# finsberg/fenicsx-beat

Measured on AMD Instinct MI355X. Metric: node_updates_per_sec, higher is better.
Workload: dtype f64

## Files before the change

### fenicsx-beat_amd/beat/_engine.py

```python

from __future__ import annotations

import ctypes as C
import os
from dataclasses import dataclass
from types import SimpleNamespace
from typing import Any

import numpy as np

from . import _hip
from ._deferred import DeferredUpdate


@dataclass
class Slab:

    nz_global: int
    rank: int = 0
    world: int = 1
    weights: Any = None

    def __post_init__(self):
        if self.world > self.nz_global:
# ... 333 lines not shown
        ptrs, amps, k = self._stim_args(stim_w, stim_amp)
        return self.deferred.solved(x, *_solve_record(lambda info, pend: self.lib.beat_pde_solve_dist(
            self.handle, comm.handle, v_prev.ptr, ptrs, amps, k, x.ptr, C.c_void_p(self.work.data_ptr()), rtol, atol, max_it,
            int(defer_flush), info, pend)))

    def set_guess_order(self, order: int) -> None:
        if isinstance(order, str):
            if order != "auto":
                raise ValueError(f"guess order must be an integer 0..4 or 'auto', got {order!r}")
            order = -1
        self.flush_pending()
        _hip.check(self.lib.beat_pde_set_guess_order(self.handle, int(order)))
        self.guess_order = int(order)

    def set_single_reduction(self, on) -> None:
        _hip.check(self.lib.beat_pde_set_single_reduction(self.handle, -1 if on is None else int(bool(on))))

    def set_small(self, enable: bool) -> None:
        _hip.check(self.lib.beat_pde_set_small_grid_solve(self.handle, int(bool(enable))))

    def small_active(self) -> bool:
        return bool(self.lib.beat_pde_small_grid_solve_active(self.handle))

    RR_ROUTE_KEYS = ("available", "ry", "pd", "by_rows_mask", "nsegx", "nrb", "zc", "nchunks", "total_blocks", "guess_ry")

    def rr_route(self) -> dict:
        out = (C.c_int * len(self.RR_ROUTE_KEYS))()
        _hip.check(self.lib.beat_pde_rr_route(self.handle, out))
        return {k: int(v) for k, v in zip(self.RR_ROUTE_KEYS, out)}

    def guess_traffic(self) -> dict:
        out = (C.c_int * 4)()
        _hip.check(self.lib.beat_pde_guess_traffic(self.handle, out))
        return {"reads": int(out[0]), "writes": int(out[1]), "order": int(out[2]), "pending": bool(out[3])}

    def guess_reset(self) -> None:
        self.flush_pending()
        _hip.check(self.lib.beat_pde_guess_reset(self.handle))

    def flush_pending(self) -> None:
        self.deferred.flush()

    def apply(self, which, x, y):
        _hip.check(self.lib.beat_pde_apply(self.handle, which, x.ptr, y.ptr))


def conductivity_array(M, mesh) -> np.ndarray:
    from . import _stencil, grid

    if isinstance(M, (grid.Function, grid.VectorFunction)):
        raise TypeError("the conductivity is a tensor: build it from a fibre field with "
                        "beat.conductivities.define_conductivity_tensor (vector P1 functions and per-cell fields are accepted)")
# ... 462 lines not shown
```

### fenicsx-beat_amd/beat/_hip.py

```python

from __future__ import annotations

import ctypes as C
import os
from pathlib import Path

_HERE = Path(__file__).resolve().parent
_LIB_PATH = Path(os.environ.get("BEAT_HIP_LIBRARY", _HERE / "lib" / "libbeat_hip.so"))

MODEL_SIMPLE_ODE = 0
MODEL_FHN_DEMO = 1
MODEL_FHN_README = 2
MODEL_TP06_GRL1 = 3
MODEL_TORORD_DYNCL_GRL1 = 4
MODEL_TORORD_LAND_GRL1 = 5
(MATH_EXP, MATH_EXP_INT, MATH_LOG, MATH_LOG_INT, MATH_RCP, MATH_RSQRT, MATH_TP06_RCP2, MATH_TP06_RCP3, MATH_TP06_RCP4,
 MATH_TORORD_RCP2, MATH_TORORD_RCP3, MATH_TORORD_RCP4, MATH_TP06_PHI_SMALL, MATH_TP06_PHI7, MATH_TORORD_PHI_SMALL,
 MATH_TORORD_PHI7, MATH_TP06_GRL1, MATH_TP06_ADVANCE, MATH_TP06_GATE, MATH_TORORD_ADVANCE, MATH_TORORD_GATE,
 MATH_TORORD_GATE_B) = range(22)
MATH_IN = (1, 1, 1, 1, 1, 1, 2, 3, 4, 2, 3, 4, 1, 1, 1, 1, 4, 4, 4, 4, 4, 4)
MATH_OUT = (1, 1, 1, 1, 1, 1, 2, 3, 4, 2, 3, 4, 1, 1, 1, 1, 1, 1, 1, 1, 1, 1)
MAX_STIM = 8
MAX_CLASSES = 32
MAX_LEADS = 16
# ... 80 lines not shown
    "beat_pde_set_timestep": (_int, [_vp, _dbl, _dbl, _dbl]),
    "beat_pde_apply": (_int, [_vp, _int, _vp, _vp]),
    "beat_pde_rhs": (_int, [_vp, _vp, C.POINTER(_vp), C.POINTER(_dbl), _int, _vp, _vp, _vp, _vp]),
    "beat_pde_cg_begin": (_int, [_vp, _vp, _dbl, _dbl, _int]),
    "beat_pde_spmv_dot": (_int, [_vp, _vp, _vp, _vp]),
    "beat_pde_spmv_dot_part": (_int, [_vp, _vp, _vp, _vp, _int]),
    "beat_pde_cg_update": (_int, [_vp, _vp, _vp, _vp, _vp, _vp]),
    "beat_pde_cg_next": (_int, [_vp, _vp, _vp, _vp]),
    "beat_pde_ring_size": (_int, []),
    "beat_pde_cg_update_r": (_int, [_vp, _vp, _vp, _vp, _int]),
    "beat_pde_cg_next_oop": (_int, [_vp, _vp, _vp, _vp, _vp]),
    "beat_pde_x_flush": (_int, [_vp, _vp, _vp, _vp, _i64, _int, _int]),
    "beat_pde_set_small_grid_solve": (_int, [_vp, _int]),
    "beat_pde_small_grid_solve_active": (_int, [_vp]),
    "beat_split_steps": (_int, [_vp, _int, _vp, _i64, _i64, _vp, _int, _int, _vp, _int, _vp, _vp, _vp, _vp, _int, _dbl, _dbl,
                                _int, _vp, _vp, _int, _vp, _vp]),
    "beat_split_steps_big": (_int, [_vp, _int, _vp, _i64, _i64, _vp, _int, _int, _vp, _vp, _int, _vp, _vp, _vp, _vp, _int, _dbl, _dbl, _int, _int,
                             C.POINTER(KspInfo), C.POINTER(_int), C.POINTER(C.c_float)]),
    "beat_pde_set_guess_order": (_int, [_vp, _int]),
    "beat_pde_set_single_reduction": (_int, [_vp, _int]),
    "beat_pde_fused_dist_pass": (_int, [_vp]),
    "beat_pde_tile_route": (_int, [_vp]),
    "beat_pde_rr_route": (_int, [_vp, C.POINTER(_int)]),
    "beat_pde_guess_reset": (_int, [_vp]),
    "beat_pde_guess_pending": (_int, [_vp]),
    "beat_pde_guess_history": (_int, [_vp, _vp, _vp, _vp]),
    "beat_pde_guess_traffic": (_int, [_vp, C.POINTER(_int)]),
    "beat_pde_set_preconditioner": (_int, [_vp, _int, _vp]),
    "beat_pde_pc_num_passes": (_int, [_vp]),
    "beat_pde_pc_pass": (_int, [_vp, _int, _vp, _vp, _vp, _vp, _vp]),
    "beat_pde_cg_first_z": (_int, [_vp, _vp, _vp, _vp]),
    "beat_pde_cg_next_z": (_int, [_vp, _vp, _vp, _vp]),
    "beat_pde_work_fields": (_int, [_vp]),
    "beat_pde_field_stride": (_i64, [_vp]),
    "beat_pde_solve": (
        _int,
        [_vp, _vp, C.POINTER(_vp), C.POINTER(_dbl), _int, _vp, _vp, _dbl, _dbl, _int, C.POINTER(KspInfo)],
    ),
    "beat_pde_solve_begin": (_int, [_vp, _vp, C.POINTER(_vp), C.POINTER(_dbl), _int, _vp, _vp, _dbl, _dbl, _int]),
    "beat_pde_solve_end": (_int, [_vp, C.POINTER(KspInfo), C.POINTER(_int)]),
    "beat_pde_solve_is_open": (_int, [_vp]),
    "beat_pde_solve_can_open": (_int, [_vp]),
    "beat_pde_solve_ex": (
        _int,
        [_vp, _vp, C.POINTER(_vp), C.POINTER(_dbl), _int, _vp, _vp, _dbl, _dbl, _int, _int, C.POINTER(KspInfo), C.POINTER(_int)],
    ),
# ... 93 lines not shown
```

### fenicsx-beat_amd/csrc/beat_pde.hip

```cpp
#include "beat_pde_internal.h"
#include "beat_pde_device.h"

#include <algorithm>
#include <cmath>
#include <cstdlib>
#include <cstring>
#include <vector>

const int beat_pde_detail::kOffsets[45] = {0, 0, 0,  1, 0, 0,  -1, 0, 0,  0, 1, 0,  0, -1, 0,  0, 0, 1,  0, 0, -1,
                          1, 1, 0,  -1, -1, 0,  0, 1, 1,  0, -1, -1,  1, 0, 1,  -1, 0, -1,
                          1, 1, 1,  -1, -1, -1};

namespace {
using namespace beat_pde_detail;

template <int TX_, int TY_>
struct Tile {
  static constexpr int TX = TX_, TY = TY_;
  static constexpr int PITCH = TX + 2;
  static constexpr int SLOT = (TY + 2) * PITCH;
  static constexpr int NLOAD = (SLOT + BEAT_BLOCK - 1) / BEAT_BLOCK;
  static constexpr int ROWS_PER_THREAD = TY / (BEAT_BLOCK / TX);
  static_assert(TX * TY == 1024 && ROWS_PER_THREAD == 4, "tile must hold 1024 nodes");
};
// ... 217 lines not shown
    __syncthreads();
  }

  if (MODE == MODE_SPMV_DOT || MODE == MODE_PC) {
    const double s0 = beat_block_sum(acc0, red);
    if (threadIdx.x == 0) a.partials[g.part_off + t] = s0;
  } else if (MODE == MODE_RHS) {
    const double s0 = beat_block_sum(acc0, red);
    const double s1 = beat_block_sum(acc1, red);
    const double s2 = beat_block_sum(acc2, red);
    if (threadIdx.x == 0) {
      a.partials[g.part_off + t] = s0;
      a.partials[BEAT_MAX_PARTIALS + g.part_off + t] = s1;
      a.partials[2 * BEAT_MAX_PARTIALS + g.part_off + t] = s2;
    }
  }
}

__global__ __launch_bounds__(BEAT_BLOCK) void reduce_partials_kernel(const double* __restrict__ partials, int count, int nsum, double* out,
                                                                     const double* st, double* counter, int then, double* roll_st,
                                                                     double rtol, double atol, double max_it, double* alpha_slot,
                                                                     double bound_c) {
  __shared__ double red[4];
  if (st != nullptr && st[STOP] != 0.0) return;
  if (counter != nullptr && threadIdx.x == 0) counter[0] += 1.0;
  for (int k = 0; k < nsum; ++k) {
    double s = 0.0;
    for (int i = threadIdx.x; i < count; i += BEAT_BLOCK) s += partials[(int64_t)k * BEAT_MAX_PARTIALS + i];
    s = beat_block_sum(s, red);
    if (threadIdx.x == 0) out[k] = s;
  }
  if (then != STEP_NONE && threadIdx.x == 0) beat_pcg_step(then, roll_st, rtol, atol, max_it, alpha_slot, bound_c);
}

__global__ void pcg_step_kernel(int kind, double* st, double rtol, double atol, double max_it, double* alpha_slot, double bound_c) {
  beat_pcg_step(kind, st, rtol, atol, max_it, alpha_slot, bound_c);
}

template <bool VAR>
__global__ __launch_bounds__(BEAT_BLOCK) void cg_update_kernel(Geom g, const double* __restrict__ st,
                                                               double* __restrict__ x,
                                                               double* __restrict__ r,
                                                               const double* __restrict__ p,
                                                               const double* __restrict__ q,
                                                               const double* __restrict__ dinv,
                                                               double dinv_i, double* __restrict__ partials) {
  __shared__ double red[4];
  if (st[STOP] != 0.0) return;
  const double alpha = st[RZ] / st[PQ];
  const int lane = threadIdx.x & 63, wave = threadIdx.x >> 6;
  const int nrows = g.ny * g.nz;
  double s_rz = 0.0, s_rr = 0.0;
  for (int row = blockIdx.x * 4 + wave; row < nrows; row += gridDim.x * 4) {
    const int iz = row / g.ny, iy = row - iz * g.ny;
    const int tyz = 3 * axis_type(iy, g.ny, 1, 1) + 9 * axis_type(iz, g.nz, g.z_lo_phys, g.z_hi_phys);
// ... 202 lines not shown
  const int TX = tile_tx, TY = 1024 / tile_tx;
  g.tiles_x = (g.nx + TX - 1) / TX;
  g.tiles_y = (g.ny + TY - 1) / TY;
  const int tiles = g.tiles_x * g.tiles_y;
  int nchunks = std::max(1, (TARGET_BLOCKS + tiles - 1) / tiles);
  nchunks = std::min(nchunks, g.nz);
  g.zc = (g.nz + nchunks - 1) / nchunks;
  g.nchunks = (g.nz + g.zc - 1) / g.zc;
  const int64_t total = (int64_t)tiles * g.nchunks;
  if (total > BEAT_MAX_PARTIALS) {
    g.nchunks = std::max(1, (int)(BEAT_MAX_PARTIALS / tiles));
    g.zc = (g.nz + g.nchunks - 1) / g.nchunks;
    g.nchunks = (g.nz + g.zc - 1) / g.zc;
  }
  BEAT_REQUIRE((int64_t)tiles * g.nchunks <= BEAT_MAX_PARTIALS, "xy plane too large: %d tiles", tiles);
  g.total = tiles * g.nchunks;
  g.z_lo = 0;
  g.z_hi = g.nz;
  g.part_off = 0;
  p->n = n[0] * n[1] * n[2];
  const int64_t rows = (int64_t)g.ny * g.nz;
  p->vec_grid = (unsigned)std::min<int64_t>(2048, std::max<int64_t>(1, (rows + 3) / 4));
  if (const char* e = std::getenv("BEAT_PCG_PREDICT_STOP")) p->predict_stop = e[0] != '0';
  std::memcpy(p->h_mass, host_mass_tab, sizeof(p->h_mass));
  std::memcpy(p->h_stiff, host_stiff_tab, sizeof(p->h_stiff));
  BEAT_HIP_CHECK(hipSetDevice(ctx->device));
  BEAT_HIP_CHECK(hipMalloc(&p->d_tabs, sizeof(double) * (4 * 27 * TABW + 32)));
  BEAT_HIP_CHECK(hipMalloc(&p->d_st, sizeof(double) * BEAT_ST_DOUBLES));
  BEAT_HIP_CHECK(hipMalloc(&p->d_alphas, sizeof(double) * PRING_MAX));
  BEAT_HIP_CHECK(hipMemsetAsync(p->d_st, 0, sizeof(double) * BEAT_ST_DOUBLES, ctx->stream));
  const int rc = upload_tables(p);
  if (rc) return rc;
  *out = p;
  return BEAT_OK;
}


extern "C" int beat_pde_set_ghost_types(beat_pde* pde, int ghost_lo_type, int ghost_hi_type) {
  BEAT_REQUIRE(pde != nullptr, "null pde");
  BEAT_REQUIRE(ghost_lo_type >= 0 && ghost_lo_type <= 2 && ghost_hi_type >= 0 && ghost_hi_type <= 2, "node types are 0, 1 or 2");
  pde->ghost_lo_tz = ghost_lo_type;
  pde->ghost_hi_tz = ghost_hi_type;
  return BEAT_OK;
}

extern "C" int beat_pde_destroy(beat_pde* pde) {
  if (pde == nullptr) return BEAT_OK;
  if (pde->open.on && pde->ctx != nullptr) (void)hipStreamSynchronize(pde->ctx->stream);
  (void)hipFree(pde->d_tabs);
  (void)hipFree(pde->d_st);
  (void)hipFree(pde->d_alphas);
  (void)hipFree(pde->d_batch_st);
  (void)hipFree(pde->guess.alloc);
  if (pde->h_st) (void)hipHostFree(pde->h_st);
  if (pde->ev_st) (void)hipEventDestroy(pde->ev_st);
  (void)hipFree(pde->v_A);
  (void)hipFree(pde->v_dinv);
  (void)hipFree(pde->v_B);
  (void)hipFree(pde->v_gc0);
  (void)hipFree(pde->v_seg);
  (void)hipFree(pde->v_segmask);
  (void)hipFree(pde->v_seg_tiled);
  (void)hipFree(pde->v_segmask_tiled);
  beat_vrr_destroy(pde);
  beat_vtl_destroy(pde);
  delete pde;
  return BEAT_OK;
}

static int upload_tables(beat_pde* pde) {
  const double C_m = pde->C_m, theta = pde->theta, dt = pde->dt;
  std::vector<double> h(4 * 27 * TABW + 32, 0.0);
  for (int t = 0; t < 27; ++t) {
    for (int k = 0; k < 15; ++k) {
// ... 601 lines not shown
```

### fenicsx-beat_amd/csrc/beat_pde_device.h

```cpp
#pragma once

namespace beat_pde_detail {

__device__ __forceinline__ int axis_type(int i, int n, int lo_phys, int hi_phys) {
  if (n == 1 && lo_phys && hi_phys) return 1;
  if (i == 0 && lo_phys) return 0;
  if (i == n - 1 && hi_phys) return 2;
  return 1;
}

__device__ __forceinline__ int xcd_block(int b, int total) {
  const int per = (total + 7) >> 3;
  return (b & 7) * per + (b >> 3);
}

__device__ __forceinline__ double from_left(double v) {
  const int lo = __builtin_amdgcn_update_dpp(0, __double2loint(v), 0x138, 0xf, 0xf, true);
  const int hi = __builtin_amdgcn_update_dpp(0, __double2hiint(v), 0x138, 0xf, 0xf, true);
  return __hiloint2double(hi, lo);
}
__device__ __forceinline__ double from_right(double v) {
  const int lo = __builtin_amdgcn_update_dpp(0, __double2loint(v), 0x130, 0xf, 0xf, true);
  const int hi = __builtin_amdgcn_update_dpp(0, __double2hiint(v), 0x130, 0xf, 0xf, true);
  return __hiloint2double(hi, lo);
}
// ... 12 lines not shown
```

### fenicsx-beat_amd/csrc/beat_pde_internal.h

```cpp
#pragma once
#include "beat_common.h"
#include "beat_pcg_scalar.h"
#include "beat_slab_parts.h"

#include <algorithm>
#include <cstdlib>
#include <vector>

namespace beat_pde_detail {

constexpr int PRING = 6;
constexpr int PRING_MAX = 12;
constexpr int TABW = 16;

extern const int kOffsets[45];

struct Geom {
  int nx, ny, nz;
  int64_t plane;
  int tiles_x, tiles_y, nchunks, zc, total;
  int z_lo_phys, z_hi_phys;
  int tile_tx;
  int z_lo, z_hi;
  int part_off;
// ... 30 lines not shown
  struct OpenSolve {
    bool on = false;
    int kind = beat_pde_detail::SOLVE_RR;
    bool pdot = false;
    double* x = nullptr;
    double* work = nullptr;
    int max_it = 0, launched = 0;
    int limit = 0;
    void* comm = nullptr;
    bool rr = false, merged = false, vpdot = false;
  } open;
  struct Part0 {
    int pass = beat_pde_detail::PASS_NONE;
    int blocks = 0;
  } part0;
  double* h_st = nullptr;
  hipEvent_t ev_st = nullptr;
  beat_ksp_info last_info{};
  int last_rc = 0;
  int ring = beat_pde_detail::PRING;
  int last_base = 0;
  bool predict_stop = true;
  double predict_c = 0.0;
  double* d_batch_st = nullptr;
  int ghost_lo_tz = 1, ghost_hi_tz = 1;
  int single_reduction = -1;
  beat_guess_state guess;
  void* vrr = nullptr;
  void* vtl = nullptr;
  bool small_enabled = true;
  int pc_ncoef = 1;
  double pc_coef[8] = {1.0};
  bool var = false;
  const double* v_mass = nullptr;
  const double* v_stiff = nullptr;
  double* v_A = nullptr;
  double* v_dinv = nullptr;
  double* v_B = nullptr;
  double* v_gc0 = nullptr;
  bool v_gc0_valid = false;
  bool v_pdot_dist = false;
  int64_t v_ld = 0;
  int* v_seg = nullptr;
  std::vector<int> h_seg;
  unsigned long long* v_segmask = nullptr;
  int* v_seg_tiled = nullptr;
// ... 160 lines not shown
```

### fenicsx-beat_amd/csrc/beat_pde_rr.hip

```cpp
#include "beat_pde_internal.h"
#include "beat_pde_device.h"

#include <algorithm>
#include <cmath>
#include <cstddef>
#include <cstdlib>

namespace {
using namespace beat_pde_detail;

constexpr int SEG = 62;

struct Coef {
  double c[15];
};

struct RGeom {
  int nx, ny, nz;
  int64_t plane;
  int ry;
  int nsegx, nrb, nchunks, zc;
  int total_waves, total_blocks;
  int z_lo_phys, z_hi_phys;
  int z_lo, z_hi;
// ... 7 lines not shown
struct RArgs {
  const double* x;
  const double* x2;
  double* y;
  double* y2;
  const double* tab;
  const double* tab2;
  const double* dinv;
  Coef ci, ci2;
  double dinv_i;
  double cm, omt_dt, dt;
  const double* w[BEAT_MAX_STIM];
  double amp[BEAT_MAX_STIM];
  int nstim;
  double* partials;
  double* st;
  double* alphas;
  int slot;
  const double* e;
  const double* taba;
  Coef cia;
};

struct RKernArgs {
  RGeom g;
  RArgs a;
  const double* X;
  const double* X2;
  double* Y;
  double* Y2;
};

#ifndef BEAT_RR_BUF
#define BEAT_RR_BUF 2
#endif
#ifndef BEAT_RR_NT
#define BEAT_RR_NT 2
#endif
__device__ __forceinline__ void rr_store(double* p, double v) {
#if BEAT_RR_NT & 2
  __builtin_nontemporal_store(v, p);
#else
  *p = v;
#endif
}
constexpr int RR_LOAD_AUX = (BEAT_RR_NT & 1) ? 2 : 0;

#ifndef BEAT_RR_ALIGN
#define BEAT_RR_ALIGN 1
#endif
__device__ __forceinline__ double from_left_h(double v, double h, int src_lane) {
  const int lo = __builtin_amdgcn_update_dpp(__builtin_amdgcn_readlane(__double2loint(h), src_lane), __double2loint(v), 0x138, 0xf, 0xf, false);
  const int hi = __builtin_amdgcn_update_dpp(__builtin_amdgcn_readlane(__double2hiint(h), src_lane), __double2hiint(v), 0x138, 0xf, 0xf, false);
  return __hiloint2double(hi, lo);
}
__device__ __forceinline__ double from_right_h(double v, double h, int src_lane) {
  const int lo = __builtin_amdgcn_update_dpp(__builtin_amdgcn_readlane(__double2loint(h), src_lane), __double2loint(v), 0x130, 0xf, 0xf, false);
  const int hi = __builtin_amdgcn_update_dpp(__builtin_amdgcn_readlane(__double2hiint(h), src_lane), __double2hiint(v), 0x130, 0xf, 0xf, false);
  return __hiloint2double(hi, lo);
}
#ifndef BEAT_RR_ALIGN_RHS
#define BEAT_RR_ALIGN_RHS 0
#endif
constexpr bool rr_aligned_mode(int mode) {
  return BEAT_RR_ALIGN == 1 && BEAT_RR_BUF != 0 && (mode == 0 || mode == 1 || mode == 3 || mode == 4 || (mode == 2 && BEAT_RR_ALIGN_RHS == 1));
}

#ifndef BEAT_RR_WAVES_RHS
#define BEAT_RR_WAVES_RHS 3
#endif
#ifndef BEAT_RR_WAVES_IT
#define BEAT_RR_WAVES_IT 1
#endif
template <int MODE, int RY, int PD, bool GUESS = false, bool PRED = false>
__global__ __launch_bounds__(BEAT_BLOCK, (GUESS && RY == 2 && PD == 1) ? BEAT_RR_WAVES_RHS : ((MODE == RR_PDOT || MODE == RR_RUPD) && PD == 1 ? BEAT_RR_WAVES_IT : 1)) void rr_kernel(RGeom g, RArgs a, const double* __restrict__ X,
                                                        const double* __restrict__ X2, double* __restrict__ Y,
                                                        double* __restrict__ Y2) {
  constexpr int NR = RY + 2;
  constexpr int NE = GUESS ? NR : 1;
  constexpr bool FORM = MODE == RR_PDOT || MODE == RR_UDOT || MODE == RR_PRUPD;
  constexpr bool OLD = MODE == RR_PDOT || MODE == RR_PRUPD;
  constexpr bool RAW = MODE == RR_UDOT || MODE == RR_PRUPD;
  constexpr int NW = RAW ? RY : 1;
  constexpr bool BUF = BEAT_RR_BUF == 1 || (BEAT_RR_BUF == 2 && (MODE != RR_RHS || BEAT_RR_ALIGN_RHS == 1));
  constexpr bool ALIGNED = rr_aligned_mode(MODE);
  static_assert(!ALIGNED || BUF, "aligned segments come with the raw-buffer loads");
  constexpr int SEGW = ALIGNED ? 64 : SEG;
  static_assert(!GUESS || MODE == RR_RHS, "the initial guess enters the right-hand side only");
  static_assert(!PRED || MODE == RR_PDOT, "the predicted-stop sums come with PDOT only");
  __shared__ double red[4];
  __shared__ double s_dinv[32];
  __shared__ double s_tab[27 * TABW];
  __shared__ double s_tab2[MODE == RR_RHS ? 27 * TABW : 1];
  __shared__ double s_taba[GUESS ? 27 * TABW : 1];
  __shared__ double s_rc[PRED ? 4 * 2 * RY * 64 : 1];
  __shared__ double s_acc[PRED ? 4 * 2 * 64 : 1];
  if (MODE != RR_RHS) {
    if (a.st[STOP] != 0.0) return;
  }
  if (PRED) s_acc[(threadIdx.x >> 6) * 128 + (threadIdx.x & 63)] = s_acc[(threadIdx.x >> 6) * 128 + 64 + (threadIdx.x & 63)] = 0.0;
// ... 332 lines not shown
      }
    }
    if (GUESS) {
#pragma unroll
      for (int r = 0; r < NE; ++r) {
        Em[r] = E0[r];
        E0[r] = Ep[r];
      }
    }
    if (RAW) {
#pragma unroll
      for (int j = 0; j < NW; ++j) Rw0[j] = Rwp[j];
    }
    }
  }
  }

  if (PRED) {
    acc1 = s_acc[(threadIdx.x >> 6) * 128 + (threadIdx.x & 63)];
    acc2 = s_acc[(threadIdx.x >> 6) * 128 + 64 + (threadIdx.x & 63)];
  }
  if (MODE == RR_PDOT && !PRED) {
    const double s0 = beat_block_sum(acc0, red);
    if (threadIdx.x == 0) a.partials[g.part_off + blockIdx.x] = s0;
  } else if (MODE == RR_RUPD) {
    const double s0 = beat_block_sum(acc0, red);
    const double s1 = beat_block_sum(acc1, red);
    if (threadIdx.x == 0) {
      a.partials[g.part_off + blockIdx.x] = s0;
      a.partials[BEAT_MAX_PARTIALS + g.part_off + blockIdx.x] = s1;
    }
  } else if (MODE == RR_PRUPD) {
  } else {
    const double s0 = beat_block_sum(acc0, red);
    const double s1 = beat_block_sum(acc1, red);
    const double s2 = beat_block_sum(acc2, red);
    if (threadIdx.x == 0) {
      a.partials[g.part_off + blockIdx.x] = s0;
      a.partials[BEAT_MAX_PARTIALS + g.part_off + blockIdx.x] = s1;
      a.partials[2 * BEAT_MAX_PARTIALS + g.part_off + blockIdx.x] = s2;
    }
  }
}

int rr_rows(int64_t nodes) {
  static const int forced = [] {
    const char* e = std::getenv("BEAT_RR_RY");
    const int v = e ? std::atoi(e) : 0;
    return (v == 2 || v == 4) ? v : 0;
  }();
  if (forced) return forced;
  return nodes >= ((int64_t)64 << 20) ? 4 : 2;
}

int rr_target_blocks(int64_t nodes) {
  if (const char* e = std::getenv("BEAT_RR_BLOCKS")) return std::max(1, std::atoi(e));
  return nodes >= ((int64_t)64 << 20) ? 4096 : 2048;
}

int rr_prefetch() {
  static const int pd = [] {
    const char* e = std::getenv("BEAT_RR_PD");
    const int v = e ? std::atoi(e) : 1;
    return (v >= 1 && v <= 3) ? v : 1;
// ... 60 lines not shown

RGeom make_geom(const beat_pde* pde) { return make_geom(pde, 0, pde->g.nz, 0); }

inline int grid_blocks(const RGeom& g) { return ((g.total_blocks + 7) / 8) * 8; }
inline int blocks_written(const RGeom& g) { return g.total_blocks > 0 ? grid_blocks(g) : 0; }

Coef interior_row(const double* tab) {
  Coef c;
  for (int k = 0; k < 15; ++k) c.c[k] = tab[13 * 15 + k];
  return c;
}

RArgs rr_operator_args(const beat_pde* pde, double* dev_st) {
  RArgs a{};
  a.tab = pde->d_tab(0);
  a.dinv = pde->d_dinv();
  a.ci = interior_row(pde->h_A);
  a.dinv_i = pde->h_dinv[13];
  a.partials = pde->ctx->d_partials;
  a.st = dev_st;
  return a;
}

template <int MODE, bool GUESS = false, bool PRED = false>
void launch_rr(const beat_pde* pde, const RGeom& g, const RArgs& a) {
  if (g.total_blocks <= 0) return;
  const dim3 grid((unsigned)grid_blocks(g)), block(BEAT_BLOCK);
  hipStream_t s = pde->ctx->stream;
#define BEAT_RR_LAUNCH(RYV, PDV) \
  BEAT_KERNEL((rr_kernel<MODE, RYV, PDV, GUESS, PRED>), grid, block, 0, s, g, a, a.x, GUESS ? a.e : a.x2, a.y, a.y2)
  const int pd = rr_prefetch();
  if (g.ry == 2) {
    if (pd == 2) BEAT_RR_LAUNCH(2, 2); else if (pd == 3) BEAT_RR_LAUNCH(2, 3); else BEAT_RR_LAUNCH(2, 1);
  } else {
    if (pd == 2) BEAT_RR_LAUNCH(4, 2); else if (pd == 3) BEAT_RR_LAUNCH(4, 3); else BEAT_RR_LAUNCH(4, 1);
  }
#undef BEAT_RR_LAUNCH
}
}

bool beat_rr_available(const beat_pde* pde) {
  if (pde->var || pde->pc_ncoef != 1) return false;
  if (const char* e = std::getenv("BEAT_RR")) {
    if (e[0] == '0') return false;
  }
  const RGeom g = make_geom(pde);
  const RGeom gb = make_geom(pde, 0, 1, 0);
  return (int64_t)grid_blocks(g) + 2 * grid_blocks(gb) <= BEAT_MAX_PARTIALS;
}

extern "C" int beat_pde_rr_route(const beat_pde* pde, int* host_out) {
  BEAT_REQUIRE(pde != nullptr && host_out != nullptr, "null argument");
  const RGeom g = make_geom(pde, 0, pde->g.nz, 0, 0, RR_PDOT);
  host_out[0] = beat_rr_available(pde) ? 1 : 0;
  host_out[1] = g.ry;
  host_out[2] = rr_prefetch();
  host_out[3] = rr_by_rows_mask();
  host_out[4] = g.nsegx;
  host_out[5] = g.nrb;
  host_out[6] = g.zc;
  host_out[7] = g.nchunks;
  host_out[8] = g.total_blocks;
  host_out[9] = rr_guess_rows();
  return BEAT_OK;
}

int beat_rr_rhs(beat_pde* pde, const double* dev_v_prev, const double* const* host_dev_stim_w, const double* host_stim_amp,
                int n_stim, double* dev_x, double* dev_r, double* dev_st, int part, const PcgStart* start) {
  BEAT_REQUIRE(start == nullptr || part < 0, "only a right-hand side in one part starts the solve");
  const GuessTerms& gt = pde->guess.cur;
  const bool guess = gt.d != nullptr && gt.use_e;
  const int rows = guess ? rr_guess_rows() : 0;
  RArgs a{};
  a.x = dev_v_prev;
  a.y = dev_r;
  a.y2 = (dev_x == dev_v_prev) ? nullptr : dev_x;
  a.tab = pde->d_tab(2);
  a.tab2 = pde->d_tab(3);
  a.dinv = pde->d_dinv();
  a.ci = interior_row(pde->h_mass);
  a.ci2 = interior_row(pde->h_stiff);
  a.dinv_i = pde->h_dinv[13];
  a.cm = pde->C_m;
  a.omt_dt = (1.0 - pde->theta) * pde->dt;
  a.dt = pde->dt;
  beat_fill_stimuli(a, host_dev_stim_w, host_stim_amp, n_stim);
  a.partials = pde->ctx->d_partials;
  a.st = dev_st;
  if (guess) {
    a.tab = pde->d_tab(1);
    a.ci = interior_row(pde->h_B);
    a.e = gt.e;
    a.taba = pde->d_tab(0);
    a.cia = interior_row(pde->h_A);
  }
  auto launch = [&](int z_lo, int z_hi, int part_off) {
    const RGeom g = make_geom(pde, z_lo, z_hi, part_off, rows, RR_RHS);
    if (guess)
      launch_rr<RR_RHS, true>(pde, g, a);
    else
      launch_rr<RR_RHS>(pde, g, a);
    return blocks_written(g);
  };
  int count = 0;
  if (int rc = beat_launch_parts(pde, PASS_RR_RHS, part, launch, &count)) return rc;
  return part == 0 ? BEAT_OK : beat_pde_launch_reduce(pde, count, 3, dev_st, nullptr, ScalarStep::begin(dev_st, start));
}

double beat_rr_predict_bound(const beat_pde* pde) {
  const Geom& f = pde->g;
  int depth = 0;
  auto chain = [&](const RGeom& g) {
    const int per_thread = (grid_blocks(g) + BEAT_BLOCK - 1) / BEAT_BLOCK;
    depth = std::max(depth, g.zc * g.ry + 8 + per_thread + 8);
  };
  chain(make_geom(pde, 0, f.nz, 0, 0, RR_RHS));
  chain(make_geom(pde, 0, f.nz, 0, 2, RR_RHS));
  chain(make_geom(pde, 0, f.nz, 0, 4, RR_RHS));
  chain(make_geom(pde, 0, f.nz, 0, 0, RR_PDOT));
  chain(make_geom(pde, 0, f.nz, 0, 0, RR_RUPD));
  return 4.0 * (2.0 * depth + 8.0) * std::ldexp(1.0, -53);
}

int beat_rr_pdot_part(beat_pde* pde, double* dev_st, const double* dev_r, const double* dev_p_old, double* dev_p_new,
                      int part, int slot) {
  const Geom& f = pde->g;
  const bool pred = slot >= 0 && pde->predict_stop && f.z_lo_phys && f.z_hi_phys;
  if (pred && pde->predict_c <= 0.0) pde->predict_c = beat_rr_predict_bound(pde);
  RArgs a = rr_operator_args(pde, dev_st);
  a.x = dev_r;
  a.x2 = dev_p_old;
  a.y = dev_p_new;
  auto launch = [&](int z_lo, int z_hi, int part_off) {
    const RGeom g = make_geom(pde, z_lo, z_hi, part_off, 0, RR_PDOT);
    if (pred)
      launch_rr<RR_PDOT, false, true>(pde, g, a);
    else
      launch_rr<RR_PDOT>(pde, g, a);
    return blocks_written(g);
  };
  int count = 0;
  if (int rc = beat_launch_parts(pde, PASS_RR_PDOT, part, launch, &count)) return rc;
  if (part == 0) return BEAT_OK;
  if (pred) {
    static_assert(RQ == PQS + 1 && QQ == PQS + 2, "the three sums are reduced into one run of slots");
    return beat_pde_launch_reduce(pde, count, 3, dev_st + PQS, dev_st,
                                  ScalarStep::with_slot(STEP_PREDICT, dev_st, pde->d_alphas + slot, pde->predict_c));
  }
  return beat_pde_launch_reduce(pde, count, 1, dev_st + PQ, dev_st);
}

int beat_rr_pdot(beat_pde* pde, double* dev_st, const double* dev_r, const double* dev_p_old, double* dev_p_new, int slot) {
  if (int rc = beat_rr_pdot_part(pde, dev_st, dev_r, dev_p_old, dev_p_new, 0, slot)) return rc;
  return beat_rr_pdot_part(pde, dev_st, dev_r, dev_p_old, dev_p_new, 1, slot);
}

int beat_rr_rupd(beat_pde* pde, double* dev_st, const double* dev_r, double* dev_r_new, const double* dev_p, int slot,
                 bool roll) {
  const RGeom g = make_geom(pde, 0, pde->g.nz, 0, 0, RR_RUPD);
  RArgs a = rr_operator_args(pde, dev_st);
  a.x = dev_p;
  a.x2 = dev_r;
  a.y = dev_r_new;
  a.alphas = pde->d_alphas;
  a.slot = slot;
  launch_rr<RR_RUPD>(pde, g, a);
  BEAT_LAUNCH_CHECK();
  return beat_pde_launch_reduce(pde, grid_blocks(g), 2, dev_st + RZN, dev_st, ScalarStep::after_update(dev_st, roll));
}

int beat_rr_udot_part(beat_pde* pde, double* dev_st, const double* dev_r, int part) {
  static_assert(RZN == PQ + 1 && RRN == PQ + 2, "the three sums travel as one all-reduce of dev_st[PQ..RRN]");
  RArgs a = rr_operator_args(pde, dev_st);
  a.x = dev_r;
  a.x2 = dev_r;
  auto launch = [&](int z_lo, int z_hi, int part_off) {
    const RGeom g = make_geom(pde, z_lo, z_hi, part_off, 0, RR_UDOT);
    launch_rr<RR_UDOT>(pde, g, a);
    return blocks_written(g);
  };
  int count = 0;
  if (int rc = beat_launch_parts(pde, PASS_RR_UDOT, part, launch, &count)) return rc;
  return part == 0 ? BEAT_OK : beat_pde_launch_reduce(pde, count, 3, dev_st + PQ, dev_st);
}

int beat_rr_prupd(beat_pde* pde, double* dev_st, const double* dev_r, const double* dev_p_old, double* dev_p_new,
                  double* dev_r_new) {
  const RGeom g = make_geom(pde, 0, pde->g.nz, 0, 0, RR_PRUPD);
  RArgs a = rr_operator_args(pde, dev_st);
  a.x = dev_r;
  a.x2 = dev_p_old;
// ... 7 lines not shown
```

### include/beat_hip.h

```cpp
#ifndef BEAT_HIP_H
#define BEAT_HIP_H

#include <stddef.h>
#include <stdint.h>

#ifdef __cplusplus
extern "C" {
#endif

#define BEAT_OK 0
#define BEAT_EINVAL -1
#define BEAT_EHIP -2
#define BEAT_ENOTCONV -3
#define BEAT_ENOMEM -4

#define BEAT_ABI_VERSION 1

#define BEAT_MODEL_SIMPLE_ODE 0
#define BEAT_MODEL_FHN_DEMO 1
#define BEAT_MODEL_FHN_README 2
#define BEAT_MODEL_TP06_GRL1 3

#define BEAT_MODEL_TORORD_DYNCL_GRL1 4
#define BEAT_MODEL_TORORD_LAND_GRL1 5
// ... 99 lines not shown
int beat_pde_cg_next(beat_pde* pde, double* dev_st, const double* dev_r, double* dev_p);

int beat_pde_ring_size(void);
int beat_pde_cg_update_r(beat_pde* pde, double* dev_st, double* dev_r, const double* dev_q, int slot);
int beat_pde_cg_next_oop(beat_pde* pde, double* dev_st, const double* dev_r, const double* dev_p_cur,
                         double* dev_p_next);
int beat_pde_x_flush(beat_pde* pde, const double* dev_st, double* dev_x, const double* dev_ring0,
                     int64_t field_stride, int ring_base, int only_if_full);

int beat_pde_set_preconditioner(beat_pde* pde, int ncoef, const double* host_coef);
int beat_pde_pc_num_passes(beat_pde* pde);
int beat_pde_pc_pass(beat_pde* pde, int j, const double* dev_r, double* dev_z, double* dev_q,
                     double* dev_st, double* dev_red);
int beat_pde_cg_first_z(beat_pde* pde, double* dev_st, const double* dev_z, double* dev_p);
int beat_pde_cg_next_z(beat_pde* pde, double* dev_st, const double* dev_z, double* dev_p);

int beat_pde_work_fields(beat_pde* pde);
int64_t beat_pde_field_stride(const beat_pde* pde);
int beat_pde_set_guess_order(beat_pde* pde, int order);
int beat_pde_set_single_reduction(beat_pde* pde, int on);
int beat_pde_fused_dist_pass(const beat_pde* pde);
int beat_pde_tile_route(const beat_pde* pde);
int beat_pde_rr_route(const beat_pde* pde, int* host_out);
int beat_pde_guess_reset(beat_pde* pde);
int beat_pde_guess_pending(const beat_pde* pde);
int beat_pde_guess_history(const beat_pde* pde, double** dev_d, double** dev_e, int* count);
int beat_pde_guess_traffic(const beat_pde* pde, int* host_out);

int beat_pde_set_small_grid_solve(beat_pde* pde, int enable);
int beat_pde_small_grid_solve_active(const beat_pde* pde);

#define BEAT_MAX_BATCH 1024
int beat_split_steps(beat_ctx* ctx, int model_id, double* dev_states, int64_t n, int64_t ld,
                     const double* host_params, int num_params, int v_index, beat_pde* pde, int n_steps,
                     const double* host_t0, const double* host_dt, const double* const* host_dev_stim_w, const double* host_stim_amp, int n_stim,
                     double rtol, double atol, int max_it, const int64_t* host_probe_idx, const double* host_probe_w,
                     int n_probe, double* dev_probe_out, beat_ksp_info* host_info);
int beat_split_steps_big(beat_ctx* ctx, int model_id, double* dev_states, int64_t n, int64_t ld, const double* host_params,
                         int num_params, int v_index, beat_pde* pde, double* dev_work, int n_steps, const double* host_t0,
                         const double* host_dt, const double* const* host_dev_stim_w, const double* host_stim_amp, int n_stim,
                         double rtol, double atol, int max_it, int pending_in, beat_ksp_info* host_info, int* host_pending,
                         float* host_ode_ms);

int beat_pde_solve_begin(beat_pde* pde, const double* dev_v_prev, const double* const* host_dev_stim_w,
                         const double* host_stim_amp, int n_stim, double* dev_x, double* dev_work, double rtol, double atol, int max_it);
int beat_pde_solve_end(beat_pde* pde, beat_ksp_info* info, int* host_pending);
// ... 92 lines not shown
```

Before: 11.34 billion.

## Fuse partial-sum reduction into stencil kernels via last-block ticket

Adds a last-block-done pattern to the RR stencil kernels: each block publishes its partial sums with atomic stores and draws a ticket, and the final block performs the cross-block reduction and the scalar PCG step inside the same launch. This removes the separate reduce_partials kernel launch per CG dot product in the single-device path. The reduction loop is also batched with eight loads in flight. The cost is an extra atomic and fence per block, a serial tail in one block, and a larger kernel argument struct.

```diff
diff --git a/fenicsx-beat_amd/beat/_engine.py b/fenicsx-beat_amd/beat/_engine.py
--- a/fenicsx-beat_amd/beat/_engine.py
+++ b/fenicsx-beat_amd/beat/_engine.py
@@ -379,12 +379,18 @@
     def small_active(self) -> bool:
         return bool(self.lib.beat_pde_small_grid_solve_active(self.handle))
 
-    RR_ROUTE_KEYS = ("available", "ry", "pd", "by_rows_mask", "nsegx", "nrb", "zc", "nchunks", "total_blocks", "guess_ry")
+    RR_ROUTE_KEYS = ("available", "ry", "pd", "by_rows_mask", "nsegx", "nrb", "zc", "nchunks", "total_blocks", "guess_ry",
+                     "inlaunch", "grid_pdot", "grid_rupd", "grid_rhs", "grid_rhs_guess")
 
     def rr_route(self) -> dict:
         out = (C.c_int * len(self.RR_ROUTE_KEYS))()
         _hip.check(self.lib.beat_pde_rr_route(self.handle, out))
         return {k: int(v) for k, v in zip(self.RR_ROUTE_KEYS, out)}
+
+    def rr_ticket(self):
+        out, st = C.c_int(-1), (C.c_double * 16)()
+        _hip.check(self.lib.beat_pde_rr_ticket(self.handle, C.byref(out), st))
+        return int(out.value), np.array(st[:], dtype=np.float64)
 
     def guess_traffic(self) -> dict:
         out = (C.c_int * 4)()
diff --git a/fenicsx-beat_amd/beat/_hip.py b/fenicsx-beat_amd/beat/_hip.py
--- a/fenicsx-beat_amd/beat/_hip.py
+++ b/fenicsx-beat_amd/beat/_hip.py
@@ -126,6 +126,7 @@
     "beat_pde_fused_dist_pass": (_int, [_vp]),
     "beat_pde_tile_route": (_int, [_vp]),
     "beat_pde_rr_route": (_int, [_vp, C.POINTER(_int)]),
+    "beat_pde_rr_ticket": (_int, [_vp, C.POINTER(_int), C.POINTER(_dbl)]),
     "beat_pde_guess_reset": (_int, [_vp]),
     "beat_pde_guess_pending": (_int, [_vp]),
     "beat_pde_guess_history": (_int, [_vp, _vp, _vp, _vp]),
diff --git a/fenicsx-beat_amd/csrc/beat_pde.hip b/fenicsx-beat_amd/csrc/beat_pde.hip
--- a/fenicsx-beat_amd/csrc/beat_pde.hip
+++ b/fenicsx-beat_amd/csrc/beat_pde.hip
@@ -263,15 +263,7 @@
                                                                      double rtol, double atol, double max_it, double* alpha_slot,
                                                                      double bound_c) {
   __shared__ double red[4];
-  if (st != nullptr && st[STOP] != 0.0) return;
-  if (counter != nullptr && threadIdx.x == 0) counter[0] += 1.0;
-  for (int k = 0; k < nsum; ++k) {
-    double s = 0.0;
-    for (int i = threadIdx.x; i < count; i += BEAT_BLOCK) s += partials[(int64_t)k * BEAT_MAX_PARTIALS + i];
-    s = beat_block_sum(s, red);
-    if (threadIdx.x == 0) out[k] = s;
-  }
-  if (then != STEP_NONE && threadIdx.x == 0) beat_pcg_step(then, roll_st, rtol, atol, max_it, alpha_slot, bound_c);
+  beat_reduce_partials(partials, count, nsum, out, st, counter, then, roll_st, rtol, atol, max_it, alpha_slot, bound_c, red);
 }
 
 __global__ void pcg_step_kernel(int kind, double* st, double rtol, double atol, double max_it, double* alpha_slot, double bound_c) {
@@ -520,6 +512,10 @@
   const int64_t rows = (int64_t)g.ny * g.nz;
   p->vec_grid = (unsigned)std::min<int64_t>(2048, std::max<int64_t>(1, (rows + 3) / 4));
   if (const char* e = std::getenv("BEAT_PCG_PREDICT_STOP")) p->predict_stop = e[0] != '0';
+  if (const char* e = std::getenv("BEAT_PCG_INLAUNCH")) p->inlaunch = std::atoi(e) & 3;
+  if (const char* e = std::getenv("BEAT_PCG_FUSE")) {
+    if (e[0] == '0') p->inlaunch = 0;
+  }
   std::memcpy(p->h_mass, host_mass_tab, sizeof(p->h_mass));
   std::memcpy(p->h_stiff, host_stiff_tab, sizeof(p->h_stiff));
   BEAT_HIP_CHECK(hipSetDevice(ctx->device));
@@ -527,6 +523,8 @@
   BEAT_HIP_CHECK(hipMalloc(&p->d_st, sizeof(double) * BEAT_ST_DOUBLES));
   BEAT_HIP_CHECK(hipMalloc(&p->d_alphas, sizeof(double) * PRING_MAX));
   BEAT_HIP_CHECK(hipMemsetAsync(p->d_st, 0, sizeof(double) * BEAT_ST_DOUBLES, ctx->stream));
+  BEAT_HIP_CHECK(hipMalloc(&p->d_ticket, sizeof(int)));
+  BEAT_HIP_CHECK(hipMemsetAsync(p->d_ticket, 0, sizeof(int), ctx->stream));
   const int rc = upload_tables(p);
   if (rc) return rc;
   *out = p;
@@ -548,6 +546,7 @@
   (void)hipFree(pde->d_tabs);
   (void)hipFree(pde->d_st);
   (void)hipFree(pde->d_alphas);
+  (void)hipFree(pde->d_ticket);
   (void)hipFree(pde->d_batch_st);
   (void)hipFree(pde->guess.alloc);
   if (pde->h_st) (void)hipHostFree(pde->h_st);
diff --git a/fenicsx-beat_amd/csrc/beat_pde_device.h b/fenicsx-beat_amd/csrc/beat_pde_device.h
--- a/fenicsx-beat_amd/csrc/beat_pde_device.h
+++ b/fenicsx-beat_amd/csrc/beat_pde_device.h
@@ -1,6 +1,23 @@
 #pragma once
+#include "beat_common.h"
+#include "beat_reduce_body.h"
 
 namespace beat_pde_detail {
+
+struct DeviceBlock {
+  static constexpr int THREADS = BEAT_BLOCK;
+  double* red;
+  __device__ __forceinline__ int tid() const { return (int)threadIdx.x; }
+  __device__ __forceinline__ double sum(double v) const { return beat_block_sum(v, red); }
+};
+
+__device__ __forceinline__ void beat_reduce_partials(const double* partials, int count, int nsum, double* out, const double* st,
+                                                     double* counter, int then, double* roll_st, double rtol, double atol,
+                                                     double max_it, double* alpha_slot, double bound_c, double* red) {
+  DeviceBlock blk{red};
+  beat_reduce_then_step(blk, partials, (int64_t)BEAT_MAX_PARTIALS, count, nsum, out, st, counter, then, roll_st, rtol, atol, max_it,
+                        alpha_slot, bound_c);
+}
 
 __device__ __forceinline__ int axis_type(int i, int n, int lo_phys, int hi_phys) {
   if (n == 1 && lo_phys && hi_phys) return 1;
diff --git a/fenicsx-beat_amd/csrc/beat_pde_internal.h b/fenicsx-beat_amd/csrc/beat_pde_internal.h
--- a/fenicsx-beat_amd/csrc/beat_pde_internal.h
+++ b/fenicsx-beat_amd/csrc/beat_pde_internal.h
@@ -76,6 +76,8 @@
   int last_base = 0;
   bool predict_stop = true;
   double predict_c = 0.0;
+  int inlaunch = 1;
+  int* d_ticket = nullptr;
   double* d_batch_st = nullptr;
   int ghost_lo_tz = 1, ghost_hi_tz = 1;
   int single_reduction = -1;
diff --git a/fenicsx-beat_amd/csrc/beat_pde_rr.hip b/fenicsx-beat_amd/csrc/beat_pde_rr.hip
--- a/fenicsx-beat_amd/csrc/beat_pde_rr.hip
+++ b/fenicsx-beat_amd/csrc/beat_pde_rr.hip
@@ -53,6 +53,19 @@
   Coef cia;
 };
 
+struct RTail {
+  int* ticket;
+  int count, nsum;
+  double* out;
+  const double* st;
+  double* counter;
+  double* step_st;
+  double rtol, atol, max_it;
+  double* alpha_slot;
+  double bound_c;
+  int then;
+};
+
 struct RKernArgs {
   RGeom g;
   RArgs a;
@@ -60,6 +73,7 @@
   const double* X2;
   double* Y;
   double* Y2;
+  RTail t;
 };
 
 #ifndef BEAT_RR_BUF
@@ -76,6 +90,9 @@
 #endif
 }
 constexpr int RR_LOAD_AUX = (BEAT_RR_NT & 1) ? 2 : 0;
+__device__ __forceinline__ void rr_store_partial(double* p, double v) {
+  __hip_atomic_store((unsigned long long*)p, (unsigned long long)__double_as_longlong(v), __ATOMIC_RELAXED, __HIP_MEMORY_SCOPE_AGENT);
+}
 
 #ifndef BEAT_RR_ALIGN
 #define BEAT_RR_ALIGN 1
@@ -106,7 +123,7 @@
 template <int MODE, int RY, int PD, bool GUESS = false, bool PRED = false>
 __global__ __launch_bounds__(BEAT_BLOCK, (GUESS && RY == 2 && PD == 1) ? BEAT_RR_WAVES_RHS : ((MODE == RR_PDOT || MODE == RR_RUPD) && PD == 1 ? BEAT_RR_WAVES_IT : 1)) void rr_kernel(RGeom g, RArgs a, const double* __restrict__ X,
                                                         const double* __restrict__ X2, double* __restrict__ Y,
-                                                        double* __restrict__ Y2) {
+                                                        double* __restrict__ Y2, RTail ) {
   constexpr int NR = RY + 2;
   constexpr int NE = GUESS ? NR : 1;
   constexpr bool FORM = MODE == RR_PDOT || MODE == RR_UDOT || MODE == RR_PRUPD;
@@ -485,13 +502,13 @@
   }
   if (MODE == RR_PDOT && !PRED) {
     const double s0 = beat_block_sum(acc0, red);
-    if (threadIdx.x == 0) a.partials[g.part_off + blockIdx.x] = s0;
+    if (threadIdx.x == 0) rr_store_partial(&a.partials[g.part_off + blockIdx.x], s0);
   } else if (MODE == RR_RUPD) {
     const double s0 = beat_block_sum(acc0, red);
     const double s1 = beat_block_sum(acc1, red);
     if (threadIdx.x == 0) {
-      a.partials[g.part_off + blockIdx.x] = s0;
-      a.partials[BEAT_MAX_PARTIALS + g.part_off + blockIdx.x] = s1;
+      rr_store_partial(&a.partials[g.part_off + blockIdx.x], s0);
+      rr_store_partial(&a.partials[BEAT_MAX_PARTIALS + g.part_off + blockIdx.x], s1);
     }
   } else if (MODE == RR_PRUPD) {
   } else {
@@ -499,10 +516,32 @@
     const double s1 = beat_block_sum(acc1, red);
     const double s2 = beat_block_sum(acc2, red);
     if (threadIdx.x == 0) {
-      a.partials[g.part_off + blockIdx.x] = s0;
-      a.partials[BEAT_MAX_PARTIALS + g.part_off + blockIdx.x] = s1;
-      a.partials[2 * BEAT_MAX_PARTIALS + g.part_off + blockIdx.x] = s2;
-    }
+      rr_store_partial(&a.partials[g.part_off + blockIdx.x], s0);
+      rr_store_partial(&a.partials[BEAT_MAX_PARTIALS + g.part_off + blockIdx.x], s1);
+      rr_store_partial(&a.partials[2 * BEAT_MAX_PARTIALS + g.part_off + blockIdx.x], s2);
+    }
+  }
+
+  if constexpr (MODE == RR_RHS || MODE == RR_PDOT || MODE == RR_RUPD) {
+    typedef const __attribute__((address_space(4))) char* KArgPtr;
+    KArgPtr ka = (KArgPtr)__builtin_amdgcn_kernarg_segment_ptr();
+    asm volatile("" : "+s"(ka));
+    const RKernArgs& k = *(const RKernArgs*)ka;
+    int* ticket = k.t.ticket;
+    if (ticket == nullptr) return;
+    if (threadIdx.x == 0) {
+      asm volatile("s_waitcnt vmcnt(0)" ::: "memory");
+      const int drawn = __hip_atomic_fetch_add(ticket, 1, __ATOMIC_RELAXED, __HIP_MEMORY_SCOPE_AGENT);
+      red[0] = drawn == (int)gridDim.x - 1 ? 1.0 : 0.0;
+    }
+    __syncthreads();
+    if (red[0] == 0.0) return;
+    __builtin_amdgcn_fence(__ATOMIC_ACQUIRE, "agent");
+    asm volatile("s_waitcnt vmcnt(0)" ::: "memory");
+    __syncthreads();
+    beat_reduce_partials(k.a.partials, k.t.count, k.t.nsum, k.t.out, k.t.st, k.t.counter, k.t.then, k.t.step_st, k.t.rtol, k.t.atol,
+                         k.t.max_it, k.t.alpha_slot, k.t.bound_c, red);
+    if (threadIdx.x == 0) __hip_atomic_store(ticket, 0, __ATOMIC_RELAXED, __HIP_MEMORY_SCOPE_AGENT);
   }
 }
 
@@ -609,13 +648,35 @@
   return a;
 }
 
+RTail rr_tail(const beat_pde* pde, int count, int nsum, double* out, const double* st, const ScalarStep& step = {}) {
+  RTail t{};
+  t.ticket = pde->d_ticket;
+  t.count = count;
+  t.nsum = nsum;
+  t.out = out;
+  t.st = st;
+  t.counter = step.counter;
+  t.step_st = step.st;
+  t.rtol = step.rtol;
+  t.atol = step.atol;
+  t.max_it = (double)step.max_it;
+  t.alpha_slot = step.alpha_slot;
+  t.bound_c = step.bound_c;
+  t.then = (int)step.kind;
+  return t;
+}
+
+bool rr_inlaunch(const beat_pde* pde, int bit = 1) {
+  return (pde->inlaunch & bit) != 0 && pde->d_ticket != nullptr && pde->g.z_lo_phys && pde->g.z_hi_phys;
+}
+
 template <int MODE, bool GUESS = false, bool PRED = false>
-void launch_rr(const beat_pde* pde, const RGeom& g, const RArgs& a) {
+void launch_rr(const beat_pde* pde, const RGeom& g, const RArgs& a, const RTail& t = {}) {
   if (g.total_blocks <= 0) return;
   const dim3 grid((unsigned)grid_blocks(g)), block(BEAT_BLOCK);
   hipStream_t s = pde->ctx->stream;
 #define BEAT_RR_LAUNCH(RYV, PDV) \
-  BEAT_KERNEL((rr_kernel<MODE, RYV, PDV, GUESS, PRED>), grid, block, 0, s, g, a, a.x, GUESS ? a.e : a.x2, a.y, a.y2)
+  BEAT_KERNEL((rr_kernel<MODE, RYV, PDV, GUESS, PRED>), grid, block, 0, s, g, a, a.x, GUESS ? a.e : a.x2, a.y, a.y2, t)
   const int pd = rr_prefetch();
   if (g.ry == 2) {
     if (pd == 2) BEAT_RR_LAUNCH(2, 2); else if (pd == 3) BEAT_RR_LAUNCH(2, 3); else BEAT_RR_LAUNCH(2, 1);
@@ -649,6 +710,19 @@
   host_out[7] = g.nchunks;
   host_out[8] = g.total_blocks;
   host_out[9] = rr_guess_rows();
+  host_out[10] = (rr_inlaunch(pde, 1) ? 1 : 0) | (rr_inlaunch(pde, 2) ? 2 : 0);
+  host_out[11] = grid_blocks(g);
+  host_out[12] = grid_blocks(make_geom(pde, 0, pde->g.nz, 0, 0, RR_RUPD));
+  host_out[13] = grid_blocks(make_geom(pde, 0, pde->g.nz, 0, 0, RR_RHS));
+  host_out[14] = grid_blocks(make_geom(pde, 0, pde->g.nz, 0, rr_guess_rows(), RR_RHS));
+  return BEAT_OK;
+}
+
+extern "C" int beat_pde_rr_ticket(const beat_pde* pde, int* host_ticket, double* host_st16) {
+  BEAT_REQUIRE(pde != nullptr && host_ticket != nullptr && pde->d_ticket != nullptr, "null argument");
+  BEAT_HIP_CHECK(hipStreamSynchronize(pde->ctx->stream));
+  BEAT_HIP_CHECK(hipMemcpy(host_ticket, pde->d_ticket, sizeof(int), hipMemcpyDeviceToHost));
+  if (host_st16) BEAT_HIP_CHECK(hipMemcpy(host_st16, pde->d_st, sizeof(double) * 16, hipMemcpyDeviceToHost));
   return BEAT_OK;
 }
 
@@ -681,17 +755,20 @@
     a.taba = pde->d_tab(0);
     a.cia = interior_row(pde->h_A);
   }
+  const bool tail = start != nullptr && rr_inlaunch(pde, 2);
   auto launch = [&](int z_lo, int z_hi, int part_off) {
     const RGeom g = make_geom(pde, z_lo, z_hi, part_off, rows, RR_RHS);
+    const RTail t = tail ? rr_tail(pde, blocks_written(g), 3, dev_st, nullptr, ScalarStep::begin(dev_st, start)) : RTail{};
     if (guess)
-      launch_rr<RR_RHS, true>(pde, g, a);
+      launch_rr<RR_RHS, true>(pde, g, a, t);
     else
-      launch_rr<RR_RHS>(pde, g, a);
+      launch_rr<RR_RHS>(pde, g, a, t);
     return blocks_written(g);
   };
   int count = 0;
   if (int rc = beat_launch_parts(pde, PASS_RR_RHS, part, launch, &count)) return rc;
-  return part == 0 ? BEAT_OK : beat_pde_launch_reduce(pde, count, 3, dev_st, nullptr, ScalarStep::begin(dev_st, start));
+  if (part == 0 || (tail && count > 0)) return BEAT_OK;
+  return beat_pde_launch_reduce(pde, count, 3, dev_st, nullptr, ScalarStep::begin(dev_st, start));
 }
 
 double beat_rr_predict_bound(const beat_pde* pde) {
@@ -718,26 +795,28 @@
   a.x = dev_r;
   a.x2 = dev_p_old;
   a.y = dev_p_new;
+  static_assert(RQ == PQS + 1 && QQ == PQS + 2, "the three sums are reduced into one run of slots");
+  const int nsum = pred ? 3 : 1;
+  double* out = dev_st + (pred ? PQS : PQ);
+  const ScalarStep step = pred ? ScalarStep::with_slot(STEP_PREDICT, dev_st, pde->d_alphas + slot, pde->predict_c) : ScalarStep{};
+  const bool tail = part < 0 && rr_inlaunch(pde);
   auto launch = [&](int z_lo, int z_hi, int part_off) {
     const RGeom g = make_geom(pde, z_lo, z_hi, part_off, 0, RR_PDOT);
+    const RTail t = tail ? rr_tail(pde, blocks_written(g), nsum, out, dev_st, step) : RTail{};
     if (pred)
-      launch_rr<RR_PDOT, false, true>(pde, g, a);
+      launch_rr<RR_PDOT, false, true>(pde, g, a, t);
     else
-      launch_rr<RR_PDOT>(pde, g, a);
+      launch_rr<RR_PDOT>(pde, g, a, t);
     return blocks_written(g);
   };
   int count = 0;
   if (int rc = beat_launch_parts(pde, PASS_RR_PDOT, part, launch, &count)) return rc;
-  if (part == 0) return BEAT_OK;
-  if (pred) {
-    static_assert(RQ == PQS + 1 && QQ == PQS + 2, "the three sums are reduced into one run of slots");
-    return beat_pde_launch_reduce(pde, count, 3, dev_st + PQS, dev_st,
-                                  ScalarStep::with_slot(STEP_PREDICT, dev_st, pde->d_alphas + slot, pde->predict_c));
-  }
-  return beat_pde_launch_reduce(pde, count, 1, dev_st + PQ, dev_st);
+  if (part == 0 || (tail && count > 0)) return BEAT_OK;
+  return beat_pde_launch_reduce(pde, count, nsum, out, dev_st, step);
 }
 
 int beat_rr_pdot(beat_pde* pde, double* dev_st, const double* dev_r, const double* dev_p_old, double* dev_p_new, int slot) {
+  if (slot >= 0 && rr_inlaunch(pde)) return beat_rr_pdot_part(pde, dev_st, dev_r, dev_p_old, dev_p_new, -1, slot);
   if (int rc = beat_rr_pdot_part(pde, dev_st, dev_r, dev_p_old, dev_p_new, 0, slot)) return rc;
   return beat_rr_pdot_part(pde, dev_st, dev_r, dev_p_old, dev_p_new, 1, slot);
 }
@@ -751,9 +830,11 @@
   a.y = dev_r_new;
   a.alphas = pde->d_alphas;
   a.slot = slot;
-  launch_rr<RR_RUPD>(pde, g, a);
+  const ScalarStep step = ScalarStep::after_update(dev_st, roll);
+  const bool tail = roll && rr_inlaunch(pde) && g.total_blocks > 0;
+  launch_rr<RR_RUPD>(pde, g, a, tail ? rr_tail(pde, grid_blocks(g), 2, dev_st + RZN, dev_st, step) : RTail{});
   BEAT_LAUNCH_CHECK();
-  return beat_pde_launch_reduce(pde, grid_blocks(g), 2, dev_st + RZN, dev_st, ScalarStep::after_update(dev_st, roll));
+  return tail ? BEAT_OK : beat_pde_launch_reduce(pde, grid_blocks(g), 2, dev_st + RZN, dev_st, step);
 }
 
 int beat_rr_udot_part(beat_pde* pde, double* dev_st, const double* dev_r, int part) {
diff --git a/fenicsx-beat_amd/csrc/beat_reduce_body.h b/fenicsx-beat_amd/csrc/beat_reduce_body.h
--- /dev/null
+++ b/fenicsx-beat_amd/csrc/beat_reduce_body.h
@@ -0,0 +1,31 @@
+#pragma once
+#include "beat_pcg_scalar.h"
+
+#include <cstdint>
+
+namespace beat_pde_detail {
+
+template <class Block>
+BEAT_PCG_FN void beat_reduce_then_step(Block& blk, const double* partials, int64_t stride, int count, int nsum, double* out,
+                                       const double* st, double* counter, int then, double* roll_st, double rtol, double atol,
+                                       double max_it, double* alpha_slot, double bound_c) {
+  if (st != nullptr && st[STOP] != 0.0) return;
+  if (counter != nullptr && blk.tid() == 0) counter[0] += 1.0;
+  for (int k = 0; k < nsum; ++k) {
+    constexpr int BATCH = 8, T = Block::THREADS;
+    const double* p = partials + (int64_t)k * stride;
+    double s = 0.0;
+    int i = blk.tid();
+    for (; i + (BATCH - 1) * T < count; i += BATCH * T) {
+      double v[BATCH];
+      for (int u = 0; u < BATCH; ++u) v[u] = p[i + u * T];
+      for (int u = 0; u < BATCH; ++u) s += v[u];
+    }
+    for (; i < count; i += T) s += p[i];
+    s = blk.sum(s);
+    if (blk.tid() == 0) out[k] = s;
+  }
+  if (then != STEP_NONE && blk.tid() == 0) beat_pcg_step(then, roll_st, rtol, atol, max_it, alpha_slot, bound_c);
+}
+
+}
diff --git a/include/beat_hip.h b/include/beat_hip.h
--- a/include/beat_hip.h
+++ b/include/beat_hip.h
@@ -145,6 +145,7 @@
 int beat_pde_fused_dist_pass(const beat_pde* pde);
 int beat_pde_tile_route(const beat_pde* pde);
 int beat_pde_rr_route(const beat_pde* pde, int* host_out);
+int beat_pde_rr_ticket(const beat_pde* pde, int* host_ticket, double* host_st16);
 int beat_pde_guess_reset(beat_pde* pde);
 int beat_pde_guess_pending(const beat_pde* pde);
 int beat_pde_guess_history(const beat_pde* pde, double** dev_d, double** dev_e, int* count);
```

New measurement: 11.39 billion, median of 6. No clear change (+0.4%).
